# GrandmasterB42/bevyray

Hardware: AMD Instinct MI355X
Metric: Mrays/s at 1920x1080, 64 spp, 8 bounces (higher is better)
Workload: dtype f32

## Files before the change

### bevyray_amd/csrc/brt_device.h

```cpp
#pragma once
#include <hip/hip_runtime.h>

#include "brt_layout.h"

namespace brt {

#define BRT_DEV __device__ __forceinline__

#if defined(BRT_INT_STEP) || defined(BRT_EXACT_FORMS) || defined(BRT_SHARED_RCP) || defined(BRT_WALK_FAST_TOP)
#error "BRT_INT_STEP, BRT_EXACT_FORMS, BRT_SHARED_RCP and BRT_WALK_FAST_TOP are retired (fixed at 7, 6, 3 and 1); their arms build from commit 6041ad3"
#endif

#ifndef BRT_LEAF_ISSUE
#define BRT_LEAF_ISSUE 15
#endif

#if defined(__HIP_DEVICE_COMPILE__) && !defined(__gfx950__)
#define BRT_HAND_ASM 0
#else
#define BRT_HAND_ASM 1
#endif

#ifndef BRT_ASM_COUNT
#define BRT_ASM_COUNT 0
#endif
struct AsmCounts { uint32_t int_exec, int_lanes, leaf_exec, leaf_lanes, ball_exec, ball_lanes, fix_int_lanes, fix_leaf_lanes, rows_int_exec, rows_calls, rows_cycles, wide_cycles, leaf_slow; };
__device__ __forceinline__ bool first_active_lane() {
    const uint64_t m = __ballot(true);
    return __builtin_amdgcn_mbcnt_hi((uint32_t)(m >> 32), __builtin_amdgcn_mbcnt_lo((uint32_t)m, 0u)) == 0u;
}

#ifndef BRT_MAT_BY_SPHERE
#define BRT_MAT_BY_SPHERE 1
#endif

constexpr float kInf = 3.40282347e+38f;

struct f3 {
    float x, y, z;
};
BRT_DEV f3 mk3(float x, float y, float z) { f3 r; r.x = x; r.y = y; r.z = z; return r; }
BRT_DEV f3 operator+(f3 a, f3 b) { return mk3(a.x + b.x, a.y + b.y, a.z + b.z); }
BRT_DEV f3 operator-(f3 a, f3 b) { return mk3(a.x - b.x, a.y - b.y, a.z - b.z); }
BRT_DEV f3 operator*(f3 a, f3 b) { return mk3(a.x * b.x, a.y * b.y, a.z * b.z); }
BRT_DEV f3 operator*(float s, f3 a) { return mk3(s * a.x, s * a.y, s * a.z); }
BRT_DEV f3 neg3(f3 a) { return mk3(-a.x, -a.y, -a.z); }
BRT_DEV float dot3(f3 a, f3 b) { return (a.x * b.x + a.y * b.y) + a.z * b.z; }
BRT_DEV float min_f(float a, float b) { return __builtin_fminf(a, b); }
BRT_DEV float max_f(float a, float b) { return __builtin_fmaxf(a, b); }
BRT_DEV float min_sel(float a, float b) { return b < a ? b : a; }
BRT_DEV float max_sel(float a, float b) { return a < b ? b : a; }

constexpr float kPlainLo = 0x1p-40f, kPlainHi = 0x1p40f;
struct RcpRef { float d, r1; };
BRT_DEV RcpRef rcp_refined(float d) {
    const float r0 = __builtin_amdgcn_rcpf(d);
    const float e = __builtin_fmaf(-d, r0, 1.0f);
    RcpRef R;
    R.d = d;
    R.r1 = __builtin_fmaf(e, r0, r0);
    return R;
}
BRT_DEV float div_plain(float n, RcpRef R) {
    float q = n * R.r1;
    float e = __builtin_fmaf(-R.d, q, n);
    q = __builtin_fmaf(e, R.r1, q);
    e = __builtin_fmaf(-R.d, q, n);
    return __builtin_fmaf(e, R.r1, q);
}
BRT_DEV float recip_plain(float d) {
    const RcpRef R = rcp_refined(d);
    float e = __builtin_fmaf(-d, R.r1, 1.0f);
    const float q = __builtin_fmaf(e, R.r1, R.r1);
    e = __builtin_fmaf(-d, q, 1.0f);
    return __builtin_fmaf(e, R.r1, q);
}
BRT_DEV bool all_within(f3 v, float lo, float hi) {
    const float ax = __builtin_fabsf(v.x), ay = __builtin_fabsf(v.y), az = __builtin_fabsf(v.z);
    return min_f(min_f(ax, ay), az) >= lo && max_f(max_f(ax, ay), az) <= hi;
}
BRT_DEV bool wave_all(bool p) { return __ballot(!p) == 0ull; }
BRT_DEV uint32_t wave_count(bool p) {
    return (uint32_t)__builtin_amdgcn_readfirstlane((int)__popcll(__ballot(p)));
}

BRT_DEV float sqrt_plain(float x) {
    const float s = __builtin_amdgcn_sqrtf(x);
    const float s_dn = __uint_as_float(__float_as_uint(s) - 1u), s_up = __uint_as_float(__float_as_uint(s) + 1u);
    const float r_dn = __builtin_fmaf(-s_dn, s, x), r_up = __builtin_fmaf(-s_up, s, x);
    float r = (0.0f >= r_dn) ? s_dn : s;
    r = (0.0f < r_up) ? s_up : r;
    return r;
}

BRT_DEV float sqrt_rsq(float x) {
    const float r = __builtin_amdgcn_rsqf(x);
    float s = x * r, h = 0.5f * r;
    const float e = __builtin_fmaf(-h, s, 0.5f);
    h = __builtin_fmaf(h, e, h);
    s = __builtin_fmaf(s, e, s);
    const float d = __builtin_fmaf(-s, s, x);
    return __builtin_fmaf(d, h, s);
}

BRT_DEV f3 sqrt3(f3 c) {
    const float ax = __builtin_fabsf(c.x), ay = __builtin_fabsf(c.y), az = __builtin_fabsf(c.z);
    const float mx = max_f(max_f(ax, ay), az);
    const bool zero = mx == 0.0f;
    const bool plain = (min_f(min_f(ax, ay), az) >= 0x1p-80f && mx <= 0x1p80f) || zero;
    if (wave_all(plain)) return mk3(sqrt_plain(c.x), sqrt_plain(c.y), sqrt_plain(c.z));
    return mk3(__builtin_sqrtf(c.x), __builtin_sqrtf(c.y), __builtin_sqrtf(c.z));
}

BRT_DEV f3 normalize3(f3 v) {
    if (wave_all(all_within(v, kPlainLo, 0x1p39f))) {
        const RcpRef R = rcp_refined(sqrt_plain(dot3(v, v)));
        return mk3(div_plain(v.x, R), div_plain(v.y, R), div_plain(v.z, R));
    }
    const float len = __builtin_sqrtf(dot3(v, v));
    return mk3(v.x / len, v.y / len, v.z / len);
}

BRT_DEV uint32_t f32_to_u32_sat(float f) {
    if (!(f > 0.0f)) return 0u;
    if (f >= 4294967296.0f) return 0xffffffffu;
    return (uint32_t)f;
}

BRT_DEV uint32_t rng_next(uint32_t state) {
    const uint32_t old = state + 747796405u + 2891336453u;
    const uint32_t word = ((old >> ((old >> 28u) + 4u)) ^ old) * 277803737u;
    return (word >> 22u) ^ word;
}
BRT_DEV float rng_float(uint32_t& state) {
    state = rng_next(state);
    return (float)state * 2.3283064365386963e-10f;
}
BRT_DEV float two_x_minus_one(float x) { return __builtin_fmaf(x, 2.0f, -1.0f); }
BRT_DEV float rng_ball_coord(uint32_t& state) {
    state = rng_next(state);
    return __builtin_fmaf((float)state, 4.656612873077392578125e-10f, -1.0f);
}
BRT_DEV f3 rng_unit_ball(uint32_t& state) {
    f3 p;
    for (;;) {
        const float x = rng_float(state);
        const float y = rng_float(state);
        const float z = rng_float(state);
        p = mk3(two_x_minus_one(x), two_x_minus_one(y), two_x_minus_one(z));
        if (dot3(p, p) <= 1.0f) break;
    }
    return p;
}

#ifndef BRT_BALL_ASM
#define BRT_BALL_ASM BRT_HAND_ASM
#endif
BRT_DEV void ball_loop_asm(uint32_t& rng, f3& acc, float rough, uint64_t m2, uint64_t m1, AsmCounts* ac = nullptr) {
#if BRT_HAND_ASM
#if BRT_ASM_COUNT
    uint32_t c_exec, c_lanes, c_tmp;
#define BRT_COUNT_BALL "s_bcnt1_i32_b64 %[c_tmp], exec\n s_add_u32 %[c_lanes], %[c_lanes], %[c_tmp]\n s_add_u32 %[c_exec], %[c_exec], 1\n"
#else
#define BRT_COUNT_BALL
#endif
    uint32_t t;
    float x, y, z, x1, y1, z1, q, r;
    uint64_t s_all, s_up, s_two, s_part;
    const uint32_t c_mul = 277803737u, c_2m31 = 0x30000000u ;
#define BRT_RNG_DRAW(dst)                                                                                                   \
    "v_add_u32_e32 %[rng], 0xd8e8c2ba, %[rng]\n"                       \
    "v_lshrrev_b32_e32 %[t], 28, %[rng]\n"                                                                                  \
    "v_add_u32_e32 %[t], 4, %[t]\n"                                                                                         \
    "v_lshrrev_b32_e32 %[t], %[t], %[rng]\n"                                                                                \
    "v_xor_b32_e32 %[rng], %[t], %[rng]\n"                                                                                  \
    "v_mul_lo_u32 %[rng], %[rng], %[c_mul]\n"                                                                               \
    "v_lshrrev_b32_e32 %[t], 22, %[rng]\n"                                                                                  \
    "v_xor_b32_e32 %[rng], %[t], %[rng]\n"                                                                                  \
    "v_cvt_f32_u32_e32 " dst ", %[rng]\n"                                                                                  \
    "v_fma_f32 " dst ", " dst ", %[c_2m31], -1.0\n"
#if BRT_LEAF_ISSUE & 8
#define BRT_BALL_BOOK                                                                                                       \
        "s_and_b64 exec, %[m2], vcc\n"                                                              \
        "s_xor_b64 %[m1], %[m1], vcc\n"                                           \
        "s_andn2_b64 %[m2], %[m2], vcc\n"
#else
#define BRT_BALL_BOOK                                                                                                       \
        "s_and_b64 %[s_up], %[m2], vcc\n"                                                           \
        "s_andn2_b64 %[m1], %[m1], vcc\n"                                                          \
        "s_andn2_b64 %[m2], %[m2], vcc\n"                                                                                   \
        "s_or_b64 %[m1], %[m1], %[s_up]\n"                                                                                  \
        "s_mov_b64 exec, %[s_up]\n"
#endif
#define BRT_BALL_ITERATION                                                                                                  \
        BRT_RNG_DRAW("%[x]")                                                                                                \
        BRT_RNG_DRAW("%[y]")                                                                                                \
        BRT_RNG_DRAW("%[z]")                                                                                                \
        "v_mul_f32_e32 %[q], %[x], %[x]\n"                                             \
        "v_mul_f32_e32 %[r], %[y], %[y]\n"                                                                                  \
        "v_add_f32_e32 %[q], %[q], %[r]\n"                                                                                  \
        "v_mul_f32_e32 %[r], %[z], %[z]\n"                                                                                  \
        "v_add_f32_e32 %[q], %[q], %[r]\n"                                                                                  \
        "v_cmp_ge_f32_e32 vcc, 1.0, %[q]\n"                                              \
        BRT_BALL_BOOK                                                                                                       \
        "v_mov_b32_e32 %[x1], %[x]\n"                                                         \
        "v_mov_b32_e32 %[y1], %[y]\n"                                                                                       \
        "v_mov_b32_e32 %[z1], %[z]\n"                                                                                       \
        "s_or_b64 exec, %[m2], %[m1]\n"
    asm volatile(
#if BRT_ASM_COUNT
        "s_mov_b32 %[c_exec], 0\n s_mov_b32 %[c_lanes], 0\n"
#endif
        "s_mov_b64 %[s_all], exec\n"
        "s_mov_b64 %[s_two], %[m2]\n"
        "s_or_b64 %[s_part], %[m2], %[m1]\n"
        "s_mov_b64 exec, %[s_part]\n"
        "s_cbranch_execz 2f\n"
        "1:\n"
        BRT_COUNT_BALL
        BRT_BALL_ITERATION
        "s_cbranch_scc1 1b\n"
        "s_mov_b64 exec, %[s_two]\n"
        "v_add_f32_e32 %[ax], %[ax], %[x1]\n"
        "v_add_f32_e32 %[ay], %[ay], %[y1]\n"
        "v_add_f32_e32 %[az], %[az], %[z1]\n"
        "s_mov_b64 exec, %[s_part]\n"
        "v_mul_f32_e32 %[x], %[rough], %[x]\n"
        "v_mul_f32_e32 %[y], %[rough], %[y]\n"
        "v_mul_f32_e32 %[z], %[rough], %[z]\n"
        "v_add_f32_e32 %[ax], %[ax], %[x]\n"
        "v_add_f32_e32 %[ay], %[ay], %[y]\n"
        "v_add_f32_e32 %[az], %[az], %[z]\n"
        "2:\n"
        "s_mov_b64 exec, %[s_all]\n"
        : [rng] "+v"(rng), [ax] "+v"(acc.x), [ay] "+v"(acc.y), [az] "+v"(acc.z), [m2] "+s"(m2), [m1] "+s"(m1),
          [t] "=&v"(t), [x] "=&v"(x), [y] "=&v"(y), [z] "=&v"(z), [x1] "=&v"(x1), [y1] "=&v"(y1), [z1] "=&v"(z1), [q] "=&v"(q), [r] "=&v"(r),
          [s_all] "=&s"(s_all), [s_up] "=&s"(s_up), [s_two] "=&s"(s_two), [s_part] "=&s"(s_part)
#if BRT_ASM_COUNT
          , [c_exec] "=&s"(c_exec), [c_lanes] "=&s"(c_lanes), [c_tmp] "=&s"(c_tmp)
#endif
        : [rough] "v"(rough), [c_mul] "s"(c_mul), [c_2m31] "s"(c_2m31)
        : "vcc", "scc", "memory");
#if BRT_ASM_COUNT
    if (first_active_lane()) { ac->ball_exec += c_exec; ac->ball_lanes += c_lanes; }
#endif
#undef BRT_COUNT_BALL
#undef BRT_BALL_ITERATION
#undef BRT_BALL_BOOK
#undef BRT_RNG_DRAW
#endif
}

BRT_DEV bool slab_push(f3 o, f3 inv, f3 bmin, f3 bmax, float closest) {
    const float tminx = (bmin.x - o.x) * inv.x, tmaxx = (bmax.x - o.x) * inv.x;
    const float tminy = (bmin.y - o.y) * inv.y, tmaxy = (bmax.y - o.y) * inv.y;
    const float tminz = (bmin.z - o.z) * inv.z, tmaxz = (bmax.z - o.z) * inv.z;
    const float t_near = max_f(max_f(min_f(tminx, tmaxx), min_f(tminy, tmaxy)), min_f(tminz, tmaxz));
    const float t_far = min_f(min_f(max_f(tminx, tmaxx), max_f(tminy, tmaxy)), max_f(tminz, tmaxz));
    const bool hit = (t_far >= t_near) && (t_far > 0.0f);
    return hit && (t_near < closest);
}

BRT_DEV void sphere_test(f3 o, f3 d, float a, float4 s, uint32_t idx, float& closest, uint32_t& closest_idx) {
    const f3 oc = mk3(s.x - o.x, s.y - o.y, s.z - o.z);
    const float h = dot3(d, oc);
    const float c = dot3(oc, oc) - s.w;
    const float disc = h * h - a * c;
    const float t = (h - __builtin_sqrtf(disc)) / a;
    const bool accept = (t > 0.001f) && (t < closest);
    closest = accept ? t : closest;
    closest_idx = accept ? idx : closest_idx;
}

BRT_DEV float float_below(float closest) { return __uint_as_float(__float_as_uint(closest) - 1u); }

struct ScenePtrs {
    const char* pairs;
    const char* pairs_far;
    uint32_t near_bytes;
    uint32_t near_base;
    uint32_t sph_base;
    uint32_t rows_scratch;
    bool boxes_ordered;
    bool spheres_bounded;
    const float4* spheres;
    const uint32_t* sphere_material;
    const float4* materials;
    const float4* sphere_mats;
    const uint2* leaf_table;
    bool minmax_select;
    uint32_t* hits;
};

struct HitCounters {
    uint32_t node_pops, interior, sphere_tests, hits;
    uint32_t sec_exec[8], sec_lanes[8];
    unsigned long long ticks_ball;
    AsmCounts asm_counts;
};
enum { SEC_INTERIOR = 0, SEC_LEAF, SEC_CAMERA, SEC_SCATTER, SEC_SKY, SEC_BALL, SEC_CAMERA_TOP, SEC_ROUND };

template <bool COUNTERS>
BRT_DEV void prof_section(HitCounters& hc, int sec, bool pred) {
    if (COUNTERS) {
        const uint64_t m = __ballot(pred);
        if (pred && __builtin_amdgcn_mbcnt_hi((uint32_t)(m >> 32), __builtin_amdgcn_mbcnt_lo((uint32_t)m, 0u)) == 0u) {
            hc.sec_exec[sec]++;
            hc.sec_lanes[sec] += (uint32_t)__popcll(m);
        }
    }
}

template <typename StackT>
struct WalkState {
    float a;
    f3 inv;
    float closest;
    uint32_t closest_idx;
    uint32_t cur;
    StackT* sp;
    uint32_t n;
    uint32_t ox, oy, oz;
};

template <bool D16, typename StackT>
BRT_DEV void walk_begin(WalkState<StackT>& w, const ScenePtrs& sc, uint32_t root_desc, StackT* stk, f3 d) {
    w.a = dot3(d, d);
    if (wave_all(all_within(d, kPlainLo, kPlainHi))) w.inv = mk3(recip_plain(d.x), recip_plain(d.y), recip_plain(d.z));
    else w.inv = mk3(1.0f / d.x, 1.0f / d.y, 1.0f / d.z);
    w.ox = PAIR_X + ((w.inv.x < 0.0f && !sc.minmax_select) ? 16u : 0u);
    w.oy = PAIR_Y + ((w.inv.y < 0.0f && !sc.minmax_select) ? 16u : 0u);
    w.oz = PAIR_Z + ((w.inv.z < 0.0f && !sc.minmax_select) ? 16u : 0u);
    w.closest = kInf;
    w.closest_idx = 0xffffffffu;
    w.cur = root_desc;
    stk[0] = (StackT)-1;
    w.sp = stk;
    w.n = 0;
}

template <bool D16, bool SIMPLE_TREE, typename StackT>
BRT_DEV bool walk_pending(const WalkState<StackT>& w) {
    return w.cur != Desc<D16>::DONE && (SIMPLE_TREE || w.n < 31u);
}

template <int STRIDE, bool COUNTERS, bool D16, bool SIMPLE_TREE, typename StackT>
BRT_DEV void walk_leaf_step(const ScenePtrs& sc, f3 o, f3 d, float a, float& closest, uint32_t& closest_idx, uint32_t& cur,
                            StackT*& sp, uint32_t& n, HitCounters& hc) {
    using DS = Desc<D16>;
    if (COUNTERS) hc.node_pops++;
    if (BRT_ASM_COUNT && !COUNTERS && STRIDE == 64) hc.asm_counts.fix_leaf_lanes++;
    if (STRIDE == 64) prof_section<COUNTERS>(hc, SEC_LEAF, true);
    const uint32_t first = cur & DS::INDEX_MASK;
    const uint32_t popped = (uint32_t)(int32_t)*sp;
    if (SIMPLE_TREE || (cur & DS::LEAF1)) {
        if (COUNTERS) hc.sphere_tests++;
        sphere_test(o, d, a, sc.spheres[first], first, closest, closest_idx);
    } else {
        const uint2 lt = sc.leaf_table[first];
        for (uint32_t i = lt.x; i < lt.x + lt.y; i++) {
            if (COUNTERS) hc.sphere_tests++;
            sphere_test(o, d, a, sc.spheres[i], i, closest, closest_idx);
        }
    }
    cur = popped;
    sp -= STRIDE;
    n--;
}

template <bool BOUNDED = false>
BRT_DEV bool ray_is_safe(f3 o, f3 inv) {
    constexpr int kFinite = 0x1F8;
    constexpr int kFiniteNonZero = 0x198;
    const bool origin = BOUNDED ? (__builtin_fabsf(o.x) <= kLeafOriginMax && __builtin_fabsf(o.y) <= kLeafOriginMax && __builtin_fabsf(o.z) <= kLeafOriginMax)
                                : (__builtin_amdgcn_classf(o.x, kFinite) && __builtin_amdgcn_classf(o.y, kFinite) && __builtin_amdgcn_classf(o.z, kFinite));
    return origin && __builtin_amdgcn_classf(inv.x, kFiniteNonZero) &&
           __builtin_amdgcn_classf(inv.y, kFiniteNonZero) && __builtin_amdgcn_classf(inv.z, kFiniteNonZero);
}

template <int STRIDE, bool COUNTERS, bool FIX, bool D16, int MODE, typename StackT, bool HITS = false, bool SEL = false>
BRT_DEV void walk_interior_step(const ScenePtrs& sc, f3 o, f3 inv, uint32_t ox, uint32_t oy, uint32_t oz, float below,
                                uint32_t& cur, StackT*& sp, uint32_t& n, HitCounters& hc) {
    if (COUNTERS) { hc.node_pops++; hc.interior++; }
    if (BRT_ASM_COUNT && !COUNTERS && STRIDE == 64) hc.asm_counts.fix_int_lanes++;
    if (HITS) atomicAdd(sc.hits + cur, 1u);
    if (STRIDE == 64) prof_section<COUNTERS>(hc, SEC_INTERIOR, true);
    const uint32_t ro = Desc<D16>::record_offset(cur);
    float4 gx, gy, gz;
    uint2 D;
    if (MODE == SCENE_LDS_TOP) {
        typedef float vf4 __attribute__((ext_vector_type(4)));
        typedef uint32_t vu2 __attribute__((ext_vector_type(2)));
        typedef const __attribute__((address_space(3))) vf4 lds_f4;
        typedef const __attribute__((address_space(3))) vu2 lds_u2;
        typedef const __attribute__((address_space(1))) vf4 glb_f4;
        typedef const __attribute__((address_space(1))) vu2 glb_u2;
        vf4 vx, vy, vz;
        vu2 vd;
        if (ro < sc.near_bytes) {
            const uint32_t rec = sc.near_base + ro;
// ... 931 lines not shown
```

### bevyray_amd/csrc/brt_trace.h

```cpp
#pragma once
#include <hip/hip_runtime.h>

#include <cstdlib>
#include <type_traits>

#include "brt_device.h"
#include "brt_kernels.h"

#ifndef BRT_PHASE_PRIO_AT
#define BRT_PHASE_PRIO_AT 2
#endif

namespace brt {

struct PixelCoord {
    uint32_t px, py;
    uint32_t local_row;
    uint32_t tile;
    uint32_t t;
    bool inside;
};
BRT_DEV uint32_t slot_tile(const FrameParams& fp, uint32_t slot_tile_index) {
    return fp.tile_order ? fp.tile_order[slot_tile_index] : slot_tile_index;
}
// ... 59 lines not shown
    SliceSlot r;
    r.f = fp.slice_state + slot;
    r.a = fp.slice_state + n + 4u * slot;
    r.b = fp.slice_state + 5u * n + 4u * slot;
    return r;
}

BRT_DEV bool slice_store(const FrameParams& fp, const PixelState& ps, uint32_t rays, bool with_b) {
    const SliceSlot rec = slice_slot(fp, ps);
    const uint32_t ready = (fp.slice_serial << 2) | kSliceReady, gave_up = (fp.slice_serial << 2) | kSliceGaveUp;
    const slice_u4 a = {ps.rng, __float_as_uint(ps.sum.x), __float_as_uint(ps.sum.y), __float_as_uint(ps.sum.z)};
    const slice_u4 b = {__float_as_uint(ps.dsum), rays, 0u, 0u};
#if BRT_SLICE_SYNC == 2
    *reinterpret_cast<slice_u4*>(rec.a) = a;
    if (with_b) *reinterpret_cast<slice_u4*>(rec.b) = b;
    return __hip_atomic_exchange(rec.f, ready, __ATOMIC_RELEASE, __HIP_MEMORY_SCOPE_AGENT) == gave_up;
#elif BRT_SLICE_SYNC == 1
    asm volatile("global_store_dwordx4 %0, %1, off sc1" :: "v"(rec.a), "v"(a) : "memory");
    if (with_b) asm volatile("global_store_dwordx4 %0, %1, off sc1" :: "v"(rec.b), "v"(b) : "memory");
    asm volatile("s_waitcnt vmcnt(0)" ::: "memory");
    return slice_xchg(rec.f, ready) == gave_up;
#else
    uint32_t seen = slice_xchg(rec.a + 0, a.x);
    seen |= slice_xchg(rec.a + 1, a.y);
    seen |= slice_xchg(rec.a + 2, a.z);
    seen |= slice_xchg(rec.a + 3, a.w);
    seen |= slice_xchg(rec.b + 0, b.x);
    seen |= slice_xchg(rec.b + 1, b.y);
    uint32_t flag = ready;
    asm volatile("v_and_b32 %1, 0, %1\n\tv_or_b32 %0, %0, %1" : "+v"(flag), "+v"(seen));
    return slice_xchg(rec.f, flag) == gave_up;
#endif
}

BRT_DEV bool slice_load(const FrameParams& fp, PixelState& ps, uint32_t* rays_before, bool with_b) {
    const SliceSlot rec = slice_slot(fp, ps);
    const uint32_t ready = (fp.slice_serial << 2) | kSliceReady, gave_up = (fp.slice_serial << 2) | kSliceGaveUp;
    slice_u4 a, b = {0u, 0u, 0u, 0u};
#if BRT_SLICE_SYNC == 2
    if (__hip_atomic_exchange(rec.f, gave_up, __ATOMIC_ACQUIRE, __HIP_MEMORY_SCOPE_AGENT) != ready) return false;
    a = *reinterpret_cast<const slice_u4*>(rec.a);
    if (with_b) b = *reinterpret_cast<const slice_u4*>(rec.b);
#elif BRT_SLICE_SYNC == 1
    if (slice_xchg(rec.f, gave_up) != ready) return false;
    asm volatile("global_load_dwordx4 %0, %1, off sc1" : "=&v"(a) : "v"(rec.a) : "memory");
    if (with_b) asm volatile("global_load_dwordx4 %0, %1, off sc1" : "+&v"(b) : "v"(rec.b) : "memory");
    asm volatile("s_waitcnt vmcnt(0)" : "+v"(a), "+v"(b) :: "memory");
#else
    if (slice_xchg(rec.f, gave_up) != ready) return false;
    a.x = slice_read(rec.a + 0); a.y = slice_read(rec.a + 1); a.z = slice_read(rec.a + 2); a.w = slice_read(rec.a + 3);
    b.x = slice_read(rec.b + 0); b.y = slice_read(rec.b + 1);
#endif
    ps.rng = a.x;
    ps.sum = mk3(__uint_as_float(a.y), __uint_as_float(a.z), __uint_as_float(a.w));
    ps.dsum = __uint_as_float(b.x);
    *rays_before = b.y;
    ps.sample = slice_point(fp);
    return true;
}

BRT_DEV void pixel_begin(const FrameParams& fp, const PixelCoord& c, PixelState& ps) {
    const float uvx = ((float)c.px + 0.5f) / (float)fp.width;
    const float uvy = ((float)c.py + 0.5f) / (float)fp.height;
    ps.rng = pixel_seed(fp, uvx, uvy);
    ps.ndc0x = uvx * 2.0f - 1.0f;
    ps.ndc0y = 1.0f - uvy * 2.0f;
    ps.sum = mk3(0.0f, 0.0f, 0.0f);
    ps.dsum = 0.0f;
    ps.sample = 0;
    ps.out_index = c.local_row * fp.width + c.px;
    ps.frame_index = fp.raster_dense ? ps.out_index : c.py * fp.width + c.px;
    ps.tile = c.tile | (c.t << kTileLaneShift);
}

template <bool PURE_LEVEL = false>
BRT_DEV void pixel_finish(const FrameParams& fp, const PixelState& ps, float* out_tile, const float* raster_rgba,
                          const float* raster_depth) {
    const f3 avg = mk3(ps.sum.x / fp.spp_f, ps.sum.y / fp.spp_f, ps.sum.z / fp.spp_f);
    if (PURE_LEVEL) {
        reinterpret_cast<float4*>(out_tile)[ps.out_index] = make_float4(avg.x, avg.y, avg.z, 1.0f);
        return;
    }
    const float avg_depth = ps.dsum / fp.spp_f;
    reinterpret_cast<float4*>(out_tile)[ps.out_index] =
        resolve_pixel(fp, avg, avg_depth, raster_rgba, raster_depth, ps.frame_index);
}

template <bool COUNTERS>
BRT_DEV bool shade_segment(const ScenePtrs& sc, const FrameParams& fp, f3& o, f3& d, f3& tput, uint32_t& bounce,
                           float& first_depth, float t, uint32_t idx, uint32_t& rng, f3& color, HitCounters& hc,
                           bool or_short_circuit = false) {
    if (bounce == 0) first_depth = t;
    f3 light = mk3(0.0f, 0.0f, 0.0f);
    bool ended;
    if (t == kInf) {
        light = background_gradient(d);
        ended = true;
    } else {
        hc.hits++;
        f3 att;
        const bool absorbed = scatter<COUNTERS>(sc, o, d, t, idx, rng, att, hc, or_short_circuit);
        if (absorbed) {
            ended = true;
        } else {
            tput = tput * att;
            bounce++;
            ended = bounce > fp.bounce_count;
            if (ended) tput = mk3(0.0f, 0.0f, 0.0f);
        }
    }
    if (ended) {
        const f3 c = tput * light;
        color = mk3(__builtin_sqrtf(c.x), __builtin_sqrtf(c.y), __builtin_sqrtf(c.z));
    }
    return ended;
}

template <bool COUNTERS, int LEAN, bool TUNABLE>
BRT_DEV void shade_landed(const ScenePtrs& sc, const FrameParams& fp, bool landed, float t, uint32_t idx, PixelState& ps,
                          f3& o, f3& d, f3& tput, uint32_t& bounce, float& first_depth, bool& active, bool& need_cam,
                          uint32_t& n_rays, HitCounters& hc, float* out_tile, const float* raster_rgba,
                          const float* raster_depth) {
    const bool osc = TUNABLE && (fp.policy_flags & 1u);
    const bool sel = TUNABLE && (fp.policy_flags & 2u);
    const bool pw5 = TUNABLE && (fp.policy_flags & 4u);
    const bool hit = landed && t != kInf, sky = landed && t == kInf;
    prof_section<COUNTERS>(hc, SEC_SCATTER, hit);
    prof_section<COUNTERS>(hc, SEC_SKY, sky);
    auto end_sample = [&](f3 c) {
        ps.sum = ps.sum + sqrt3(c);
        if (!LEAN) ps.dsum = ps.dsum + (first_depth == kInf ? fp.fallback_far : first_depth);
        ps.sample++;
        bounce = 0;
        need_cam = true;
        if (ps.sample == ps.sample_end) {
            const uint32_t at_end = ps.tile >> kSliceShift, tile = ps.tile & kTileMask;
            if (at_end == kSliceFirst) {
                ps.tile |= kSliceDone << kSliceShift;
            } else {
                const uint32_t rays = n_rays - ps.rays_begin;
                pixel_finish<LEAN != 0>(fp, ps, out_tile, raster_rgba, raster_depth);
                if (fp.tile_cost) {
                    atomicAdd(&fp.tile_cost[tile], rays);
                    atomicMax(&fp.tile_cost[fp.local_strips * fp.tiles_x + tile], rays);
                }
            }
            active = false;
        }
    };
    if (!landed) return;
    n_rays++;
    if (bounce == 0) first_depth = t;
    f3 v1 = d;
    if (hit) {
        hc.hits++;
        const float4 s = sc.spheres[idx];
        o = mk3(o.x + t * d.x, o.y + t * d.y, o.z + t * d.z);
        v1 = mk3(o.x - s.x, o.y - s.y, o.z - s.z);
    }
    const f3 n1 = normalize3(v1);
    bool metal = false, glass = false, diffuse = false, absorbed = false;
    f3 att, acc;
    float ior, draw;
    if (hit) {
#if BRT_MAT_BY_SPHERE
        const float4 m0 = sc.sphere_mats[2 * idx];
        const float4 m1 = sc.sphere_mats[2 * idx + 1];
#else
        const uint32_t mid = sc.sphere_material[idx];
        const float4 m0 = sc.materials[2 * mid];
        const float4 m1 = sc.materials[2 * mid + 1];
#endif
        metal = rng_float(ps.rng) < m0.w;
        glass = !metal && (rng_float(ps.rng) < m1.w);
        diffuse = !metal && !glass;
        if (glass && !osc) draw = rng_float(ps.rng);
        ior = m1.z;
        att = glass ? mk3(1.0f, 1.0f, 1.0f) : mk3(m0.x, m0.y, m0.z);
        uint32_t need = metal ? 1u : (diffuse ? 2u : 0u);
        acc = diffuse ? n1 : mk3(-0.0f, -0.0f, -0.0f);
        float scale = diffuse ? 1.0f : m1.x;
        unsigned long long t_ball = 0;
        if (COUNTERS) t_ball = wall_clock64();
        if (BRT_BALL_ASM && !COUNTERS) {
            ball_loop_asm(ps.rng, acc, m1.x, __builtin_amdgcn_ballot_w64(diffuse), __builtin_amdgcn_ballot_w64(metal), &hc.asm_counts);
            need = 0u;
        }
        while (need != 0u) {
            if (COUNTERS) prof_section<COUNTERS>(hc, SEC_BALL, true);
            const float px = rng_ball_coord(ps.rng);
            const float py = rng_ball_coord(ps.rng);
            const float pz = rng_ball_coord(ps.rng);
            const f3 p = mk3(px, py, pz);
            const bool ok = dot3(p, p) <= 1.0f;
            const f3 cand = acc + scale * p;
            acc = mk3(ok ? cand.x : acc.x, ok ? cand.y : acc.y, ok ? cand.z : acc.z);
            scale = ok ? m1.x : scale;
            need -= ok ? 1u : 0u;
        }
        if (COUNTERS) {
            const uint64_t m = __ballot(true);
            if (mbcnt64(m) == 0u) hc.ticks_ball += wall_clock64() - t_ball;
        }
        if (diffuse) {
            const float eps = 1e-8f;
            if (__builtin_fabsf(acc.x) < eps && __builtin_fabsf(acc.y) < eps && __builtin_fabsf(acc.z) < eps) acc = n1;
            absorbed = dot3(acc, n1) < 0.0f;
        }
    }
    const bool limit = hit && bounce >= fp.bounce_count;
    const bool early = sky || (diffuse && (absorbed || limit)) || (glass && limit && !osc);
    bool cam = false;
    f3 cdir;
    if (early) {
        f3 c;
        if (sky) {
            const float a = 0.5f * (n1.y + 1.0f);
            const float b = 1.0f - a;
            c = tput * mk3(b * 1.0f + a * 0.5f, b * 1.0f + a * 0.7f, b * 1.0f + a * 1.0f);
        } else if (absorbed) {
            c = tput * mk3(0.0f, 0.0f, 0.0f);
        } else {
            c = mk3(0.0f, 0.0f, 0.0f);
        }
        end_sample(c);
        cam = active;
        if (cam) {
            prof_section<COUNTERS>(hc, SEC_CAMERA, true);
            cdir = camera_dir_raw(fp, ps.ndc0x, ps.ndc0y, ps.rng);
        }
    }
    const bool second = (metal || glass) && !early;
    if (second || cam) {
        const float dn = dot3(d, n1);
        f3 v2 = metal ? d - (2.0f * dn) * n1 : d;
        if (cam) v2 = cdir;
        const f3 u = normalize3(v2);
        if (cam) {
            d = u;
            need_cam = false;
        } else if (metal) {
            d = u + acc;
            absorbed = dot3(d, n1) < 0.0f;
        } else {
            const float ri = dn < 0.0f ? (1.0f / ior) : ior;
            const float cos_theta = sel ? min_sel(dot3(neg3(u), n1), 1.0f) : min_f(dot3(neg3(u), n1), 1.0f);
            const float sin_theta = __builtin_sqrtf(1.0f - cos_theta * cos_theta);
            const bool cannot_refract = ri * sin_theta > 1.0f;
            const float refl = schlick(cos_theta, ri, pw5);
            bool reflects = cannot_refract;
            if (osc) {
                if (!cannot_refract) reflects = refl > rng_float(ps.rng);
            } else {
                reflects = reflects || (refl > draw);
            }
            d = reflects ? reflect3(u, n1) : refract3(u, n1, ri, sel);
        }
    }
    if (hit && !early) {
        if (diffuse) d = acc;
        if (absorbed || limit) {
            f3 c = mk3(0.0f, 0.0f, 0.0f);
            if (absorbed) c = tput * c;
            end_sample(c);
        } else {
            tput = tput * att;
            bounce++;
        }
    }
}

BRT_DEV void pool_lock(uint32_t* ctl, uint32_t lane) {
    if (lane == 0)
        while (atomicCAS(&ctl[0], 0u, 1u) != 0u) __builtin_amdgcn_s_sleep(1);
    __builtin_amdgcn_fence(__ATOMIC_ACQUIRE, "workgroup");
}
BRT_DEV void pool_unlock(uint32_t* ctl, uint32_t lane) {
    __builtin_amdgcn_fence(__ATOMIC_RELEASE, "workgroup");
    if (lane == 0) atomicExch(&ctl[0], 0u);
}
BRT_DEV uint32_t pool_peek(const uint32_t* ctl, int i) { return __atomic_load_n(&ctl[i], __ATOMIC_RELAXED); }


#ifndef BRT_PRIO_TOP
#define BRT_PRIO_TOP 1
#endif
template <int MODE, bool D16, bool SIMPLE, bool COUNTERS, bool TUNABLE, int LEAN>
__global__ __launch_bounds__(BRT_BLOCK) void k_trace_persistent(DeviceSceneView sv, FrameParams fp,
                                                                uint32_t* __restrict__ queue_counter,
                                                                float* __restrict__ out_tile,
                                                                const float* __restrict__ raster_rgba,
                                                                const float* __restrict__ raster_depth,
                                                                unsigned long long* __restrict__ counters) {
    static_assert(MODE == SCENE_GLOBAL || D16, "a scene staged in LDS always uses 16-bit descriptors");
    static_assert(!LEAN || (!COUNTERS && !TUNABLE), "LEAN is a specialisation of the production timing kernel");
    using StackT = typename std::conditional<D16, int16_t, int32_t>::type;
    extern __shared__ uint4 smem[];
    ScenePtrs sc;
    StackT* stacks;
    sc.materials = reinterpret_cast<const float4*>(sv.materials);
    sc.sphere_mats = reinterpret_cast<const float4*>(sv.sphere_mats);
    sc.boxes_ordered = sv.boxes_ordered != 0u;
    sc.spheres_bounded = sv.spheres_bounded != 0u;
    sc.pairs_far = reinterpret_cast<const char*>(sv.pairs);
    sc.near_bytes = 0u;
    sc.near_base = 0u;
    sc.sph_base = 0u;
    sc.rows_scratch = 0u;
    sc.hits = nullptr;
    sc.minmax_select = TUNABLE && (fp.policy_flags & 2u) != 0u;
    if (MODE == SCENE_LDS) {
        const uint32_t pair_granules = (uint32_t)(pair_array_bytes(sv.n_pairs) / 16);
        float4* p = reinterpret_cast<float4*>(smem);
        float4* l_pairs = p; p += pair_granules;
        float4* l_sp = p; p += sv.n_models;
        uint2* p2 = reinterpret_cast<uint2*>(p);
        uint2* l_lt = p2; p2 += sv.n_leaf_table;
        uint32_t* p1 = reinterpret_cast<uint32_t*>(p2);
        uint32_t* l_sm = p1; p1 += BRT_MAT_BY_SPHERE ? 0u : sv.n_models;
        stacks = reinterpret_cast<StackT*>(p1);
        const float4* g_pairs = reinterpret_cast<const float4*>(sv.pairs);
        const float4* g_sp = reinterpret_cast<const float4*>(sv.spheres);
        const uint2* g_lt = reinterpret_cast<const uint2*>(sv.leaf_table);
        for (uint32_t i = threadIdx.x; i < pair_granules; i += blockDim.x) l_pairs[i] = g_pairs[i];
        for (uint32_t i = threadIdx.x; i < sv.n_models; i += blockDim.x) { l_sp[i] = g_sp[i]; if (!BRT_MAT_BY_SPHERE) l_sm[i] = sv.sphere_material[i]; }
        for (uint32_t i = threadIdx.x; i < sv.n_leaf_table; i += blockDim.x) l_lt[i] = g_lt[i];
        sc.pairs = reinterpret_cast<const char*>(l_pairs);
        sc.near_base = (uint32_t)(uintptr_t)(__attribute__((address_space(3))) char*)reinterpret_cast<char*>(l_pairs);
        sc.sph_base = (uint32_t)(uintptr_t)(__attribute__((address_space(3))) char*)reinterpret_cast<char*>(l_sp);
        sc.spheres = l_sp; sc.sphere_material = BRT_MAT_BY_SPHERE ? sv.sphere_material : l_sm; sc.leaf_table = l_lt;
    } else {
        sc.spheres = reinterpret_cast<const float4*>(sv.spheres);
        sc.sphere_material = sv.sphere_material;
        sc.leaf_table = reinterpret_cast<const uint2*>(sv.leaf_table);
        if (MODE == SCENE_LDS_TOP) {
            const uint32_t pair_granules = sv.lds_pairs * PAIR_UNITS;
            float4* l_pairs = reinterpret_cast<float4*>(smem);
            const float4* g_pairs = reinterpret_cast<const float4*>(sv.pairs);
// ... 440 lines not shown
```

Baseline: 37210.

## Hoist material fetch ahead of hit-point math and compute ball masks in asm

Under the default BRT_SHADE_FETCH=5, per-sphere material loads are issued right after the sphere load, before the hit-point and normal math, so their latency overlaps that arithmetic (only when BRT_MAT_BY_SPHERE is set). The metal and diffuse lane masks for the rejection-sampling ball loop are now computed inside the asm with v_cmp on the lottery values, replacing the two separate ballot builtins. An optional bit-8 path folds the first accepted sample directly into the accumulator instead of staging it in copies. An uninitialised u_glass placeholder is fed to the asm for metal lanes, which relies on those lanes being excluded by the metal mask.

After: 37360, median of 6. About the same (+0.4%).

```diff
diff --git a/bevyray_amd/csrc/brt_device.h b/bevyray_amd/csrc/brt_device.h
--- a/bevyray_amd/csrc/brt_device.h
+++ b/bevyray_amd/csrc/brt_device.h
@@ -13,6 +13,10 @@
 
 #ifndef BRT_LEAF_ISSUE
 #define BRT_LEAF_ISSUE 15
+#endif
+
+#ifndef BRT_SHADE_FETCH
+#define BRT_SHADE_FETCH 5
 #endif
 
 #if defined(__HIP_DEVICE_COMPILE__) && !defined(__gfx950__)
@@ -156,7 +160,8 @@
 #ifndef BRT_BALL_ASM
 #define BRT_BALL_ASM BRT_HAND_ASM
 #endif
-BRT_DEV void ball_loop_asm(uint32_t& rng, f3& acc, float rough, uint64_t m2, uint64_t m1, AsmCounts* ac = nullptr) {
+struct BallLottery { float u_metal, metallic, u_glass, transmission; };
+BRT_DEV void ball_loop_asm(uint32_t& rng, f3& acc, float rough, uint64_t m2, uint64_t m1, const BallLottery& lot, AsmCounts* ac = nullptr) {
 #if BRT_HAND_ASM
 #if BRT_ASM_COUNT
     uint32_t c_exec, c_lanes, c_tmp;
@@ -165,8 +170,12 @@
 #define BRT_COUNT_BALL
 #endif
     uint32_t t;
-    float x, y, z, x1, y1, z1, q, r;
-    uint64_t s_all, s_up, s_two, s_part;
+    float x, y, z, q, r;
+    uint64_t s_all, s_up, s_part;
+#if !(BRT_SHADE_FETCH & 8)
+    float x1, y1, z1;
+    uint64_t s_two;
+#endif
     const uint32_t c_mul = 277803737u, c_2m31 = 0x30000000u ;
 #define BRT_RNG_DRAW(dst)                                                                                                   \
     "v_add_u32_e32 %[rng], 0xd8e8c2ba, %[rng]\n"                       \
@@ -203,16 +212,39 @@
         "v_add_f32_e32 %[q], %[q], %[r]\n"                                                                                  \
         "v_cmp_ge_f32_e32 vcc, 1.0, %[q]\n"                                              \
         BRT_BALL_BOOK                                                                                                       \
+        BRT_BALL_FIRST                                                                                                      \
+        "s_or_b64 exec, %[m2], %[m1]\n"
+#if BRT_SHADE_FETCH & 8
+#define BRT_BALL_FIRST                                                                                                      \
+        "v_add_f32_e32 %[ax], %[ax], %[x]\n"                         \
+        "v_add_f32_e32 %[ay], %[ay], %[y]\n"                                                                                \
+        "v_add_f32_e32 %[az], %[az], %[z]\n"
+#define BRT_BALL_FIRST_SUM
+#else
+#define BRT_BALL_FIRST                                                                                                      \
         "v_mov_b32_e32 %[x1], %[x]\n"                                                         \
         "v_mov_b32_e32 %[y1], %[y]\n"                                                                                       \
-        "v_mov_b32_e32 %[z1], %[z]\n"                                                                                       \
-        "s_or_b64 exec, %[m2], %[m1]\n"
+        "v_mov_b32_e32 %[z1], %[z]\n"
+#define BRT_BALL_FIRST_SUM                                                                                                  \
+        "s_mov_b64 exec, %[s_two]\n"                                             \
+        "v_add_f32_e32 %[ax], %[ax], %[x1]\n"                                                                               \
+        "v_add_f32_e32 %[ay], %[ay], %[y1]\n"                                                                               \
+        "v_add_f32_e32 %[az], %[az], %[z1]\n"
+#endif
     asm volatile(
 #if BRT_ASM_COUNT
         "s_mov_b32 %[c_exec], 0\n s_mov_b32 %[c_lanes], 0\n"
 #endif
         "s_mov_b64 %[s_all], exec\n"
+#if BRT_SHADE_FETCH & 4
+        "v_cmp_lt_f32_e64 %[m1], %[u_metal], %[metallic]\n"
+        "v_cmp_lt_f32_e64 %[m2], %[u_glass], %[transmission]\n"
+        "s_or_b64 %[m2], %[m2], %[m1]\n"
+        "s_andn2_b64 %[m2], %[s_all], %[m2]\n"
+#endif
+#if !(BRT_SHADE_FETCH & 8)
         "s_mov_b64 %[s_two], %[m2]\n"
+#endif
         "s_or_b64 %[s_part], %[m2], %[m1]\n"
         "s_mov_b64 exec, %[s_part]\n"
         "s_cbranch_execz 2f\n"
@@ -220,10 +252,7 @@
         BRT_COUNT_BALL
         BRT_BALL_ITERATION
         "s_cbranch_scc1 1b\n"
-        "s_mov_b64 exec, %[s_two]\n"
-        "v_add_f32_e32 %[ax], %[ax], %[x1]\n"
-        "v_add_f32_e32 %[ay], %[ay], %[y1]\n"
-        "v_add_f32_e32 %[az], %[az], %[z1]\n"
+        BRT_BALL_FIRST_SUM
         "s_mov_b64 exec, %[s_part]\n"
         "v_mul_f32_e32 %[x], %[rough], %[x]\n"
         "v_mul_f32_e32 %[y], %[rough], %[y]\n"
@@ -233,19 +262,36 @@
         "v_add_f32_e32 %[az], %[az], %[z]\n"
         "2:\n"
         "s_mov_b64 exec, %[s_all]\n"
-        : [rng] "+v"(rng), [ax] "+v"(acc.x), [ay] "+v"(acc.y), [az] "+v"(acc.z), [m2] "+s"(m2), [m1] "+s"(m1),
-          [t] "=&v"(t), [x] "=&v"(x), [y] "=&v"(y), [z] "=&v"(z), [x1] "=&v"(x1), [y1] "=&v"(y1), [z1] "=&v"(z1), [q] "=&v"(q), [r] "=&v"(r),
-          [s_all] "=&s"(s_all), [s_up] "=&s"(s_up), [s_two] "=&s"(s_two), [s_part] "=&s"(s_part)
+        : [rng] "+v"(rng), [ax] "+v"(acc.x), [ay] "+v"(acc.y), [az] "+v"(acc.z),
+#if BRT_SHADE_FETCH & 4
+          [m2] "=&s"(m2), [m1] "=&s"(m1),
+#else
+          [m2] "+s"(m2), [m1] "+s"(m1),
+#endif
+          [t] "=&v"(t), [x] "=&v"(x), [y] "=&v"(y), [z] "=&v"(z),
+#if !(BRT_SHADE_FETCH & 8)
+          [x1] "=&v"(x1), [y1] "=&v"(y1), [z1] "=&v"(z1),
+#endif
+          [q] "=&v"(q), [r] "=&v"(r), [s_all] "=&s"(s_all), [s_up] "=&s"(s_up),
+#if !(BRT_SHADE_FETCH & 8)
+          [s_two] "=&s"(s_two),
+#endif
+          [s_part] "=&s"(s_part)
 #if BRT_ASM_COUNT
           , [c_exec] "=&s"(c_exec), [c_lanes] "=&s"(c_lanes), [c_tmp] "=&s"(c_tmp)
 #endif
         : [rough] "v"(rough), [c_mul] "s"(c_mul), [c_2m31] "s"(c_2m31)
+#if BRT_SHADE_FETCH & 4
+          , [u_metal] "v"(lot.u_metal), [metallic] "v"(lot.metallic), [u_glass] "v"(lot.u_glass), [transmission] "v"(lot.transmission)
+#endif
         : "vcc", "scc", "memory");
 #if BRT_ASM_COUNT
     if (first_active_lane()) { ac->ball_exec += c_exec; ac->ball_lanes += c_lanes; }
 #endif
 #undef BRT_COUNT_BALL
 #undef BRT_BALL_ITERATION
+#undef BRT_BALL_FIRST
+#undef BRT_BALL_FIRST_SUM
 #undef BRT_BALL_BOOK
 #undef BRT_RNG_DRAW
 #endif
diff --git a/bevyray_amd/csrc/brt_trace.h b/bevyray_amd/csrc/brt_trace.h
--- a/bevyray_amd/csrc/brt_trace.h
+++ b/bevyray_amd/csrc/brt_trace.h
@@ -235,9 +235,17 @@
     n_rays++;
     if (bounce == 0) first_depth = t;
     f3 v1 = d;
+#if BRT_MAT_BY_SPHERE && (BRT_SHADE_FETCH & 1)
+    float4 fetched_m0, fetched_m1;
+#endif
     if (hit) {
         hc.hits++;
         const float4 s = sc.spheres[idx];
+#if BRT_MAT_BY_SPHERE && (BRT_SHADE_FETCH & 1)
+        fetched_m0 = sc.sphere_mats[2 * idx];
+        fetched_m1 = sc.sphere_mats[2 * idx + 1];
+        asm volatile("" ::: "memory");
+#endif
         o = mk3(o.x + t * d.x, o.y + t * d.y, o.z + t * d.z);
         v1 = mk3(o.x - s.x, o.y - s.y, o.z - s.z);
     }
@@ -246,7 +254,9 @@
     f3 att, acc;
     float ior, draw;
     if (hit) {
-#if BRT_MAT_BY_SPHERE
+#if BRT_MAT_BY_SPHERE && (BRT_SHADE_FETCH & 1)
+        const float4 m0 = fetched_m0, m1 = fetched_m1;
+#elif BRT_MAT_BY_SPHERE
         const float4 m0 = sc.sphere_mats[2 * idx];
         const float4 m1 = sc.sphere_mats[2 * idx + 1];
 #else
@@ -254,8 +264,18 @@
         const float4 m0 = sc.materials[2 * mid];
         const float4 m1 = sc.materials[2 * mid + 1];
 #endif
-        metal = rng_float(ps.rng) < m0.w;
-        glass = !metal && (rng_float(ps.rng) < m1.w);
+        BallLottery lot;
+        lot.metallic = m0.w;
+        lot.transmission = m1.w;
+        lot.u_metal = rng_float(ps.rng);
+        metal = lot.u_metal < lot.metallic;
+#if BRT_SHADE_FETCH & 4
+        asm("" : "=v"(lot.u_glass));
+#endif
+        if (!metal) {
+            lot.u_glass = rng_float(ps.rng);
+            glass = lot.u_glass < lot.transmission;
+        }
         diffuse = !metal && !glass;
         if (glass && !osc) draw = rng_float(ps.rng);
         ior = m1.z;
@@ -266,7 +286,11 @@
         unsigned long long t_ball = 0;
         if (COUNTERS) t_ball = wall_clock64();
         if (BRT_BALL_ASM && !COUNTERS) {
-            ball_loop_asm(ps.rng, acc, m1.x, __builtin_amdgcn_ballot_w64(diffuse), __builtin_amdgcn_ballot_w64(metal), &hc.asm_counts);
+#if BRT_SHADE_FETCH & 4
+            ball_loop_asm(ps.rng, acc, m1.x, 0, 0, lot, &hc.asm_counts);
+#else
+            ball_loop_asm(ps.rng, acc, m1.x, __builtin_amdgcn_ballot_w64(diffuse), __builtin_amdgcn_ballot_w64(metal), lot, &hc.asm_counts);
+#endif
             need = 0u;
         }
         while (need != 0u) {
```
